# tohinz/multiple-objects-gan

Hardware: AMD Instinct MI355X
Metric: images/sec per G+D train step, 256x256 coco-attngan (higher is better)
Workload: dtype f32

## Files before the change

### include/mogan_hip.h

```cpp
#ifndef MOGAN_HIP_H
#define MOGAN_HIP_H

#include <stddef.h>
#include <stdint.h>

#ifdef __cplusplus
extern "C" {
#endif

typedef struct ihipStream_t* hipStream_t;

#define MOGAN_ERR_SHAPE (-1)
#define MOGAN_ERR_LAUNCH (-2)
#define MOGAN_ERR_WS (-3)

#define MOGAN_ACT_NONE 0
#define MOGAN_ACT_RELU 1
#define MOGAN_ACT_LRELU 2
#define MOGAN_ACT_GLU 3
#define MOGAN_ACT_TANH 4
#define MOGAN_ACT_SIGMOID 5

int mogan_abi_version(void);
int mogan_gemm_set_split_target(int blocks);
// ... 1 lines not shown

int mogan_gemm_tune_set(int mode, int M, int N, int K, int nz, int cfg, int split);
int mogan_gemm_tune_clear(void);

int mogan_reserve_streams(int n);

int mogan_gemm_debug_force(int cfg, int split);
int mogan_gemm_group_min_tiles(int tiles);
int mogan_mfma_form(void);

int mogan_prof_enable(int on);
int mogan_prof_collect(double* out, int max_rows);
int mogan_prof_dump(const char* path);

int mogan_conv2d_out_dims(int Hs, int Ws, int KH, int KW, int stride, int ph, int pw, int up, int* OH, int* OW);
int mogan_conv2d_fwd(const float* x, const float* w, float* y, int B, int Cin, int Hs, int Ws, int Cout, int KH,
                     int KW, int stride, int ph, int pw, int up, void* ws, size_t ws_bytes, hipStream_t stream);
int mogan_logits_head_fwd(const float* x, const float* w, const float* bias, float* p, int B, int K, int Cout,
                          hipStream_t stream);
int mogan_logits_head_bwd(const float* dp, const float* p, const float* x, const float* w, float* dx, float* dw, float* db,
                          int B, int K, int Cout, int accumulate, hipStream_t stream);
int mogan_conv2d_lrelu_fwd(const float* x, const float* w, float* z, int B, int Cin, int Hs, int Ws, int Cout, int KH, int KW,
                           int stride, int ph, int pw, float slope, void* ws, size_t ws_bytes, hipStream_t stream);
int mogan_conv2d_affine_fwd(const float* x, const float* w, const float* scale, const float* shift, float* y, int B,
                            int Cin, int Hs, int Ws, int Cout, int KH, int KW, int stride, int ph, int pw, int relu,
                            void* ws, size_t ws_bytes, hipStream_t stream);
int mogan_affine_relu_bwd_out(const float* y, const float* dy, const float* scale, float* dx, int B, int C, int HW,
                              hipStream_t stream);
typedef struct MoganConvFwdArgs {
    const float* x; long long x_bstride; const float* w; const float* scale; const float* shift;
    float* y; long long y_bstride; float* y2; long long y2_bstride; int msplit;
    int B, Cin, Hs, Ws, Cout, KH, KW, stride, ph, pw, relu;
} MoganConvFwdArgs;
typedef struct MoganConvDgradArgs {
    const float* dy; long long dy_bstride; const float* w; float* dx; long long dx_bstride;
    const float* relu_of; long long relu_bstride; int accumulate;
    int B, Cin, Hs, Ws, Cout, KH, KW, stride, ph, pw;
} MoganConvDgradArgs;
int mogan_conv2d_affine_fwd_group(int n, const MoganConvFwdArgs* args, void* ws, size_t ws_bytes, hipStream_t stream);
int mogan_conv2d_dgrad_group(int n, const MoganConvDgradArgs* args, void* ws, size_t ws_bytes, hipStream_t stream);
int mogan_conv2d_affine_fwd_ex(const float* x, long long x_bstride, const float* w, const float* scale, const float* shift,
                               float* y, long long y_bstride, float* y2, long long y2_bstride, int msplit, int B, int Cin,
                               int Hs, int Ws, int Cout, int KH, int KW, int stride, int ph, int pw, int relu, void* ws,
                               size_t ws_bytes, hipStream_t stream);
int mogan_conv2d_fwd_ex(const float* x, long long x_bstride, const float* w, float* y, long long y_bstride,
                        const float* relu_of, long long relu_bstride, int accumulate, int B, int Cin, int Hs, int Ws,
// ... 295 lines not shown
```

### multiple-objects-gan_amd/csrc/mogan_smallc.hip

```cpp
#include <hip/hip_runtime.h>
#include <stdint.h>
#include <stdlib.h>
#include "../../include/mogan_hip.h"
#include "mogan_internal.h"

namespace {

constexpr int TR = 8, TC = 32;

template <int NC, int NT, int HH, int WW>
__device__ __forceinline__ void halo_load(float (&v)[(NC * HH * WW + NT - 1) / NT], const float* __restrict__ base, size_t plane,
                                          int nvalid, int y0, int x0, int H, int W, int tid) {
    constexpr int TOT = NC * HH * WW, NE = (TOT + NT - 1) / NT;
#pragma unroll
    for (int j = 0; j < NE; ++j) {
        const int e = tid + NT * j;
        const int c = e / (HH * WW), r = e - c * (HH * WW);
        const int hy = r / WW, hx = r - hy * WW;
        const int iy = y0 + hy, ix = x0 + hx;
        const bool ok = e < TOT && c < nvalid && (unsigned)iy < (unsigned)H && (unsigned)ix < (unsigned)W;
        const float t = base[ok ? (size_t)c * plane + (size_t)iy * W + ix : 0];
        v[j] = ok ? t : 0.f;
    }
}
template <int NC, int NT, int HH, int WW, int WP>
__device__ __forceinline__ void halo_store(float (*Xs)[HH][WP], const float (&v)[(NC * HH * WW + NT - 1) / NT], int tid) {
    constexpr int TOT = NC * HH * WW, NE = (TOT + NT - 1) / NT;
#pragma unroll
    for (int j = 0; j < NE; ++j) {
        const int e = tid + NT * j;
        const int c = e / (HH * WW), r = e - c * (HH * WW);
        const int hy = r / WW, hx = r - hy * WW;
        if (e < TOT) Xs[c][hy][hx] = v[j];
    }
}
template <int NC, int NT, int HH, int WW, int WP>
__device__ __forceinline__ void stage_halo(float (*Xs)[HH][WP], const float* __restrict__ base, size_t plane, int nvalid, int y0,
                                           int x0, int H, int W, int tid) {
    float v[(NC * HH * WW + NT - 1) / NT];
    halo_load<NC, NT, HH, WW>(v, base, plane, nvalid, y0, x0, H, W, tid);
    halo_store<NC, NT, HH, WW, WP>(Xs, v, tid);
}

template <int COUT>
// ... 135 lines not shown
    stage_halo<COUT, 256, HH, WW, WP>(Ys, dy + (size_t)b * COUT * plane, plane, COUT, ty * TR - 1, tx * TC - 1, H, W, tid);
    __syncthreads();
    float r[COUT][9];
#pragma unroll
    for (int co = 0; co < COUT; ++co)
#pragma unroll
        for (int kh = 0; kh < 3; ++kh)
#pragma unroll
            for (int kw = 0; kw < 3; ++kw) r[co][kh * 3 + kw] = Ys[co][ly + 2 - kh][lx + 2 - kw];
    const bool inside = iy < H && ix < W;
    float* out = dx + (size_t)b * Cin * plane + (size_t)iy * W + ix;
    for (int ci = 0; ci < Cin; ++ci) {
        float s = 0.f;
#pragma unroll
        for (int co = 0; co < COUT; ++co) {
            const float* wc = w + ((size_t)co * Cin + ci) * 9;
#pragma unroll
            for (int k = 0; k < 9; ++k) s = fmaf(r[co][k], wc[k], s);
        }
        if (inside) out[(size_t)ci * plane] = s;
    }
}

template <int CIN>
__global__ __launch_bounds__(256) void sc_dgrad_k4s2(const float* __restrict__ dy, const float* __restrict__ w,
                                                     float* __restrict__ dx, int Cout, int H, int W, int OH, int OW,
                                                     int tiles_x, int tiles_y) {
    constexpr int CK = 8, HH = TR + 2, WW = TC + 2, WP = WW + 1;
    __shared__ float Ys[CK][HH][WP];
    int t = blockIdx.x;
    const int tx = t % tiles_x; t /= tiles_x;
    const int ty = t % tiles_y; const int b = t / tiles_y;
    const int tid = threadIdx.x, ly = tid >> 5, lx = tid & 31;
    const int Y = ty * TR + ly, X = tx * TC + lx;
    const size_t oplane = (size_t)OH * OW;
    float acc[CIN][2][2];
#pragma unroll
    for (int ci = 0; ci < CIN; ++ci) acc[ci][0][0] = acc[ci][0][1] = acc[ci][1][0] = acc[ci][1][1] = 0.f;
    float pre[(CK * HH * WW + 255) / 256];
    halo_load<CK, 256, HH, WW>(pre, dy + (size_t)b * Cout * oplane, oplane, Cout, ty * TR - 1, tx * TC - 1, OH, OW, tid);
    for (int c0 = 0; c0 < Cout; c0 += CK) {
        halo_store<CK, 256, HH, WW, WP>(Ys, pre, tid);
        __syncthreads();
        if (c0 + CK < Cout)
            halo_load<CK, 256, HH, WW>(pre, dy + ((size_t)b * Cout + c0 + CK) * oplane, oplane, Cout - c0 - CK, ty * TR - 1, tx * TC - 1, OH,
                                       OW, tid);
        const int nc = min(CK, Cout - c0);
        for (int c = 0; c < nc; ++c) {
            float d[3][3];
#pragma unroll
            for (int a = 0; a < 3; ++a)
#pragma unroll
                for (int bb = 0; bb < 3; ++bb) d[a][bb] = Ys[c][ly + a][lx + bb];
            const float* wc = w + (size_t)(c0 + c) * CIN * 16;
#pragma unroll
            for (int ci = 0; ci < CIN; ++ci) {
                const float* k = wc + ci * 16;
#pragma unroll
                for (int py = 0; py < 2; ++py)
#pragma unroll
                    for (int px = 0; px < 2; ++px) {
                        const int kh0 = py ? 0 : 1, a0 = py ? 2 : 1, kh1 = py ? 2 : 3, a1 = py ? 1 : 0;
                        const int kw0 = px ? 0 : 1, b0 = px ? 2 : 1, kw1 = px ? 2 : 3, b1 = px ? 1 : 0;
                        float s = acc[ci][py][px];
                        s = fmaf(d[a0][b0], k[kh0 * 4 + kw0], s);
                        s = fmaf(d[a0][b1], k[kh0 * 4 + kw1], s);
                        s = fmaf(d[a1][b0], k[kh1 * 4 + kw0], s);
                        s = fmaf(d[a1][b1], k[kh1 * 4 + kw1], s);
                        acc[ci][py][px] = s;
// ... 312 lines not shown
        return hipGetLastError() == hipSuccess ? 1 : MOGAN_ERR_LAUNCH;
    }
    if (up != 0 || ph != 1 || pw != 1) return 0;
    if (KH == 3 && KW == 3 && stride == 1 && Cout >= 1 && Cout <= 4) {
        const int tiles_x = cdiv(Ws, TC), tiles_y = cdiv(Hs, TR);
        const long long nb = (long long)B * tiles_x * tiles_y;
        if (nb > 0x7fffffffLL) return 0;
        dim3 grid((unsigned)nb);
        switch (Cout) {
            case 1: hipLaunchKernelGGL(sc_dgrad3x3<1>, grid, dim3(256), 0, st, dy, w, dx, Cin, Hs, Ws, tiles_x, tiles_y); break;
            case 2: hipLaunchKernelGGL(sc_dgrad3x3<2>, grid, dim3(256), 0, st, dy, w, dx, Cin, Hs, Ws, tiles_x, tiles_y); break;
            case 3: hipLaunchKernelGGL(sc_dgrad3x3<3>, grid, dim3(256), 0, st, dy, w, dx, Cin, Hs, Ws, tiles_x, tiles_y); break;
            default: hipLaunchKernelGGL(sc_dgrad3x3<4>, grid, dim3(256), 0, st, dy, w, dx, Cin, Hs, Ws, tiles_x, tiles_y); break;
        }
        return hipGetLastError() == hipSuccess ? 1 : MOGAN_ERR_LAUNCH;
    }
    if (KH == 4 && KW == 4 && stride == 2 && Cin >= 1 && Cin <= 4 && (Hs % 2) == 0 && (Ws % 2) == 0 &&
        (((uintptr_t)dx) & 7) == 0) {
        const int tiles_x = cdiv(OW, TC), tiles_y = cdiv(OH, TR);
        const long long nb = (long long)B * tiles_x * tiles_y;
        if (nb > 0x7fffffffLL) return 0;
        dim3 grid((unsigned)nb);
        switch (Cin) {
            case 1: hipLaunchKernelGGL(sc_dgrad_k4s2<1>, grid, dim3(256), 0, st, dy, w, dx, Cout, Hs, Ws, OH, OW, tiles_x, tiles_y); break;
            case 2: hipLaunchKernelGGL(sc_dgrad_k4s2<2>, grid, dim3(256), 0, st, dy, w, dx, Cout, Hs, Ws, OH, OW, tiles_x, tiles_y); break;
            case 3: hipLaunchKernelGGL(sc_dgrad_k4s2<3>, grid, dim3(256), 0, st, dy, w, dx, Cout, Hs, Ws, OH, OW, tiles_x, tiles_y); break;
            default: hipLaunchKernelGGL(sc_dgrad_k4s2<4>, grid, dim3(256), 0, st, dy, w, dx, Cout, Hs, Ws, OH, OW, tiles_x, tiles_y); break;
        }
        return hipGetLastError() == hipSuccess ? 1 : MOGAN_ERR_LAUNCH;
    }
    return 0;
}

int mogan_smallc_wgrad_try(const float* dy, const float* x, float* dw, const MoganConvShape& g, int accumulate, void* ws,
                           size_t ws_bytes, hipStream_t st) {
    const int B = g.B, Cin = g.Cin, Hs = g.Hs, Ws = g.Ws, Cout = g.Cout, KH = g.KH, KW = g.KW;
    if (is_full_map(g) && (long long)Cout * Cin * KH * KW < (1ll << 30)) {
        const int K = Cin * KH * KW;
        hipLaunchKernelGGL(sc_dot_wgrad, dim3((unsigned)cdiv(Cout * K, 256)), dim3(256), 0, st, dy, x, dw, K, Cout, B, accumulate);
        return hipGetLastError() == hipSuccess ? 1 : MOGAN_ERR_LAUNCH;
    }
    if (!(mogan_is_k33(g) && g.up == 0 && Cout >= 1 && Cout <= 4)) return 0;
    const int tiles_x = cdiv(Ws, TC), tiles_y = cdiv(Hs, TR);
    const long long nblk = (long long)B * tiles_y;
    const int n = Cout * Cin * 9;
    if (nblk > 65535 || !ws || ws_bytes < (size_t)nblk * n * sizeof(float)) return 0;
    float* part = (float*)ws;
    dim3 grid((unsigned)nblk, (unsigned)cdiv(Cin, 8));
    switch (Cout) {
        case 1: hipLaunchKernelGGL(sc_wgrad3x3<1>, grid, dim3(192), 0, st, dy, x, part, Cin, Hs, Ws, tiles_x, tiles_y); break;
        case 2: hipLaunchKernelGGL(sc_wgrad3x3<2>, grid, dim3(192), 0, st, dy, x, part, Cin, Hs, Ws, tiles_x, tiles_y); break;
        case 3: hipLaunchKernelGGL(sc_wgrad3x3<3>, grid, dim3(192), 0, st, dy, x, part, Cin, Hs, Ws, tiles_x, tiles_y); break;
        default: hipLaunchKernelGGL(sc_wgrad3x3<4>, grid, dim3(192), 0, st, dy, x, part, Cin, Hs, Ws, tiles_x, tiles_y); break;
    }
    hipLaunchKernelGGL(sc_wgrad_reduce, dim3((unsigned)cdiv(n, 4)), dim3(256), 0, st, (const float*)part, dw, n, (int)nblk,
                       accumulate);
    return hipGetLastError() == hipSuccess ? 1 : MOGAN_ERR_LAUNCH;
}

extern "C" {

int mogan_logits_head_fwd(const float* x, const float* w, const float* bias, float* p, int B, int K, int Cout,
                          hipStream_t stream) {
    if (!x || !w || !p) return MOGAN_ERR_SHAPE;
    if (B <= 0 || K <= 0 || (K & 3) || Cout < 1 || Cout > 4 || ((((uintptr_t)x) | ((uintptr_t)w)) & 15)) return MOGAN_ERR_SHAPE;
    hipLaunchKernelGGL(logits_head_fwd_kernel, dim3((unsigned)(B * Cout)), dim3(256), 0, stream, x, w, bias, p, K, Cout);
    return hipGetLastError() == hipSuccess ? 0 : MOGAN_ERR_LAUNCH;
}

int mogan_logits_head_bwd(const float* dp, const float* p, const float* x, const float* w, float* dx, float* dw, float* db,
                          int B, int K, int Cout, int accumulate, hipStream_t stream) {
    if (!dp || !p || !x || !w) return MOGAN_ERR_SHAPE;
    if (B <= 0 || K <= 0 || Cout < 1 || Cout > 4 || (long long)B * K >= (1ll << 31)) return MOGAN_ERR_SHAPE;
    const unsigned nbx = dx ? (unsigned)(((long long)B * K + 255) / 256) : 0u;
    const unsigned nbw = dw ? (unsigned)((Cout * K + 255) / 256) : 0u;
    const unsigned nbb = db ? 1u : 0u;
    if (nbx + nbw + nbb == 0) return 0;
    hipLaunchKernelGGL(logits_head_bwd_kernel, dim3(nbx + nbw + nbb), dim3(256), 0, stream, dp, p, x, w, dx, dw, db, B, K, Cout,
                       accumulate, nbx, nbw);
    return hipGetLastError() == hipSuccess ? 0 : MOGAN_ERR_LAUNCH;
}

}
```

### multiple-objects-gan_amd/csrc/mogan_stem.hip

```cpp
#include <hip/hip_runtime.h>
#include <stdint.h>
#include <stdlib.h>
#include <algorithm>
#include "../../include/mogan_hip.h"
#include "mogan_internal.h"
#include "mogan_mma.h"

#if MOGAN_X6
namespace {

typedef float f32x16 __attribute__((ext_vector_type(16)));
typedef float f32x2 __attribute__((ext_vector_type(2)));

template <int TM>
__global__ __launch_bounds__(256, 2) void stem_k4s2_lrelu_kernel(const float* __restrict__ X, const float* __restrict__ w,
                                                              float* __restrict__ Y, int H, int W, int Cout, int OH, int OW,
                                                              float slope, int ngroups, unsigned x_bytes, unsigned y_bytes) {
    constexpr int ROWS = TM * 32;
    __shared__ __attribute__((aligned(16))) uint4 As[3 * 3 * 2 * ROWS];
    const int tid = threadIdx.x, lane = tid & 63, wave = tid >> 6, h = lane >> 5, l31 = lane & 31;
    for (int e = tid; e < ROWS * 3 * 2; e += 256) {
        const int hh = e & 1, c = (e >> 1) % 3, row = e / 6;
        float v[8];
#pragma unroll
// ... 57 lines not shown
        for (int t = 0; t < TM; ++t)
#pragma unroll
            for (int r16 = 0; r16 < 16; ++r16) {
                const int m = t * 32 + (r16 & 3) + 8 * (r16 >> 2);
                float s = acc[t][r16];
                s = s > 0.f ? s : s * slope;
                if (m < Cout) __builtin_amdgcn_raw_buffer_store_b32(__builtin_bit_cast(unsigned, s), rY, vo, (unsigned)m * (unsigned)plane * 4u, 0);
            }
    };
    int g = blockIdx.x * 4 + wave;
    if (g < ngroups) load(g, va);
    while (g < ngroups) {
        const int g1 = g + nwaves;
        if (g1 < ngroups) load(g1, vb);
        compute(g, va);
        if (g1 >= ngroups) break;
        const int g2 = g1 + nwaves;
        if (g2 < ngroups) load(g2, va);
        compute(g1, vb);
        g = g2;
    }
}

}
#endif

int mogan_stem_fwd_try(const float* x, const float* w, float* y, const MoganConvShape& g, float slope, hipStream_t st) {
#if MOGAN_X6
    constexpr int on = 1;
    if (!on) return 0;
    const int B = g.B, H = g.H, W = g.W, Cout = g.Cout, OH = g.OH, OW = g.OW;
    if (!(g.Cin == 3 && mogan_is_k44(g)) || (H & 1) || (W & 1) || B <= 0) return 0;
    if ((OW & 31) || Cout < 32 || Cout > 128 || (Cout & 7) || (((uintptr_t)x) & 7) || !(slope > 0.f)) return 0;
    if ((long long)B * 3 * H * W >= (1ll << 29) || (long long)B * Cout * OH * OW >= (1ll << 30)) return 0;
    const long long ngroups = (long long)B * OH * (OW / 32);
    if (ngroups > 0x7fffffffLL) return 0;
    static int ncu = 0;
    if (!ncu) {
        int dev = 0; hipDeviceProp_t pr;
        if (hipGetDevice(&dev) == hipSuccess && hipGetDeviceProperties(&pr, dev) == hipSuccess) ncu = pr.multiProcessorCount;
        if (ncu <= 0) ncu = 256;
    }
    const int tm = (Cout + 31) / 32;
    const unsigned nblk = (unsigned)std::min<long long>((ngroups + 3) / 4, 2ll * ncu);
    const unsigned xb = 4u * (unsigned)B * 3u * (unsigned)H * (unsigned)W, yb = 4u * (unsigned)B * Cout * OH * OW;
#define MOGAN_STEM_CASE(T) case T: hipLaunchKernelGGL((stem_k4s2_lrelu_kernel<T>), dim3(nblk), dim3(256), 0, st, x, w, y, H, W, Cout, OH, \
                                                      OW, slope, (int)ngroups, xb, yb); break;
    switch (tm) {
// ... 13 lines not shown
```

### multiple-objects-gan_amd/hip/lib.py

```python
import contextlib
import ctypes
import os

import torch

_HERE = os.path.dirname(os.path.dirname(os.path.abspath(__file__)))
LIB_PATH = os.environ.get("MOGAN_LIB") or os.path.join(_HERE, "libmogan_hip.so")

P, I, F, L, Z, D = ctypes.c_void_p, ctypes.c_int, ctypes.c_float, ctypes.c_longlong, ctypes.c_size_t, ctypes.c_double

SIGNATURES = {
    "mogan_abi_version": [],
    "mogan_gemm_set_split_target": [I],
    "mogan_stream_set_split_target": [P, I],
    "mogan_gemm_debug_force": [I, I],
    "mogan_gemm_group_min_tiles": [I],
    "mogan_mfma_form": [],
    "mogan_gemm_tune_set": [I, I, I, I, I, I, I],
    "mogan_gemm_tune_clear": [],
    "mogan_reserve_streams": [ctypes.c_int],
    "mogan_prof_enable": [I],
    "mogan_prof_collect": [P, I],
    "mogan_prof_dump": [ctypes.c_char_p],
    "mogan_conv2d_out_dims": [I, I, I, I, I, I, I, I, P, P],
    "mogan_conv2d_fwd": [P, P, P] + [I] * 11 + [P, Z, P],
    "mogan_logits_head_fwd": [P, P, P, P, I, I, I, P],
    "mogan_logits_head_bwd": [P, P, P, P, P, P, P, I, I, I, I, P],
    "mogan_conv2d_lrelu_fwd": [P, P, P] + [I] * 10 + [F, P, Z, P],
    "mogan_conv2d_affine_fwd": [P, P, P, P, P] + [I] * 11 + [P, Z, P],
    "mogan_affine_relu_bwd_out": [P, P, P, P, I, I, I, P],
    "mogan_conv2d_dgrad": [P, P, P] + [I] * 11 + [P, Z, P],
    "mogan_conv2d_wgrad": [P, P, P] + [I] * 12 + [P, Z, P],
    "mogan_wino_prep_bytes": [I] * 12,
    "mogan_wino_prep_group": [I, P, P, P, P, P, P],
    "mogan_conv_prep_bytes": [I] * 12,
    "mogan_conv_prep_group": [I, P, P, P, P, P, P, P],
    "mogan_conv2d_fwd_wp": [P, P, P, P] + [I] * 11 + [P, Z, P],
    "mogan_conv2d_dgrad_wp": [P, P, P, P] + [I] * 11 + [P, Z, P],
    "mogan_pk_conv_eligible": [I] * 11,
    "mogan_pk_weight_bytes": [I] * 6,
    "mogan_pk_weight_pack": [P, P] + [I] * 8 + [P],
    "mogan_pk_weight_pack_both": [P, P, P] + [I] * 7 + [P],
    "mogan_pk_adam_pack_both": [P] * 7 + [I] * 7 + [F, F, F, F, I, P, I, F, F, I, P],
    "mogan_conv2d_fwd_pk": [P, P, P] + [I] * 10 + [P, Z, P],
    "mogan_conv2d_dgrad_pk": [P, P, P] + [I] * 10 + [P, Z, P],
    "mogan_pk_debug_force": [I, I, I],
    "mogan_pk_wgrad_eligible": [I] * 10 + [Z],
    "mogan_conv2d_wgrad_pk": [P, P, P] + [I] * 11 + [P, Z, P],
    "mogan_pk_panel_bytes": [I, I, I],
    "mogan_deep_block_eligible": [I] * 12,
    "mogan_deep_conv_bn_act_fwd": [P] * 11 + [I] * 10 + [F, F, I, F, I, P, Z, P],
# ... 114 lines not shown
class ConvFwdArgs(ctypes.Structure):
    _fields_ = [("x", P), ("x_bstride", L), ("w", P), ("scale", P), ("shift", P), ("y", P), ("y_bstride", L), ("y2", P),
                ("y2_bstride", L), ("msplit", I)] + [(k, I) for k in ("B", "Cin", "Hs", "Ws", "Cout", "KH", "KW", "stride",
                                                                      "ph", "pw", "relu")]


class ConvDgradArgs(ctypes.Structure):
    _fields_ = [("dy", P), ("dy_bstride", L), ("w", P), ("dx", P), ("dx_bstride", L), ("relu_of", P), ("relu_bstride", L),
                ("accumulate", I)] + [(k, I) for k in ("B", "Cin", "Hs", "Ws", "Cout", "KH", "KW", "stride", "ph", "pw")]


class PkArgs(ctypes.Structure):
    _fields_ = [("wpk", P), ("panel", P), ("raw", P)] + [(k, I) for k in ("B", "M", "Cp", "CGp", "cg0", "PH", "PW", "outH", "outW",
                                                                       "KH", "KW", "stride", "ph", "pw", "dgrad", "nsplit")]


class TailArgs(ctypes.Structure):
    _fields_ = [("src", P * 3), ("src_bs", L * 3), ("src_slab", L * 3), ("src_nsplit", I * 3), ("nsrc", I), ("add", P), ("add_bs", L),
                ("mask", P), ("mask_bs", L), ("scale", P), ("shift", P), ("relu", I), ("box", I), ("dst", P), ("dst_bs", L),
                ("panel", P), ("CGp", I), ("cg0", I), ("B", I), ("n", I), ("H", I), ("W", I)]


_RESTYPE = {"mogan_bn_ws_bytes": Z, "mogan_upconv3x3_ws_bytes": Z, "mogan_pk_weight_bytes": Z, "mogan_pk_panel_bytes": Z,
            "mogan_wino_prep_bytes": Z, "mogan_conv_prep_bytes": Z, "mogan_poly3_mmd_ws_bytes": Z,
            "mogan_knn_sqdist_ws_bytes": Z, "mogan_ball_count_ws_bytes": Z, "mogan_swd_moments_ws_bytes": Z,
            "mogan_ssim_level_ws_bytes": Z, "mogan_knn_cross_ws_bytes": Z, "mogan_radial_power_ws_bytes": Z}
_ERRORS = {-1: "MOGAN_ERR_SHAPE", -2: "MOGAN_ERR_LAUNCH", -3: "MOGAN_ERR_WS"}

_lib = None
_ws = {}
WORKSPACE_BYTES = int(os.environ.get("MOGAN_WS_MB", "256")) << 20


class MoganHipError(RuntimeError):
    pass


def load():
    global _lib
    if _lib is None:
        if not os.path.isfile(LIB_PATH):
            raise MoganHipError(
                "libmogan_hip.so is not built (%s). Run `python __graft_entry__.py` / "
                "`python multiple-objects-gan_amd/build.py`; there is no CPU fallback." % LIB_PATH)
        lib = ctypes.CDLL(LIB_PATH)
        for name, args in SIGNATURES.items():
# ... 112 lines not shown
```

### multiple-objects-gan_amd/hip/ops.py

```python
import contextlib
import ctypes
import os

import torch

from . import lib
from .lib import call, ptr, stream_ptr, workspace

ACT_NONE, ACT_RELU, ACT_LRELU, ACT_GLU, ACT_TANH, ACT_SIGMOID = 0, 1, 2, 3, 4, 5

ACT_TRACE = None


BN_DEFER = None


def bn_apply_deferred(pending):
    for mean, invstd, n, rm, rv, eps, momentum in pending:
        if rm is not None or rv is not None:
            call("mogan_bn_running_update", ptr(mean), ptr(invstd), ptr(rm), ptr(rv), mean.numel(), int(n), float(eps),
                 float(momentum), stream_ptr())
    del pending[:]


# ... 69 lines not shown
    return True


def overwrite_drop(ptrs):
    for p in ptrs:
        _OVERWRITE.pop(p, None)
    del ptrs[:]


def overwrite_stale(g):
    rec = _OVERWRITE.get(g.data_ptr())
    return rec is not None and rec[1] != rec[0][0]


def _first_of_round(g):
    rec = _OVERWRITE.get(g.data_ptr()) if _OVERWRITE else None
    if rec is None:
        return False
    first = rec[1] != rec[0][0]
    rec[1] = rec[0][0]
    return first


def _wgrad_launch(dy, x, w_shape, geom, g):
    stride, ph, pw, up = geom
    acc = not _first_of_round(g)
    if WGRAD_SIDE_STREAM:
        cur, side = _wgrad_stream()
        side.wait_stream(cur)
        with torch.cuda.stream(side):
            conv2d_wgrad(dy, x, w_shape, stride, ph, pw, up, out=g, accumulate=acc)
        fr = _wgrad_frames[-1]
        if side not in fr.used:
            fr.used.append(side)
        fr.keep.append((dy, x))
        _grad_hit(g, side)
    else:
        conv2d_wgrad(dy, x, w_shape, stride, ph, pw, up, out=g, accumulate=acc)
        _grad_hit(g)


def _wgrad_accumulate(dy, x, w, geom, g):
    K = dy.shape[0] * dy.shape[2] * dy.shape[3]
    if not (MERGE_WGRAD and _wgrad_ctx_depth > 0 and K <= _MERGE_K and w.numel() >= _MERGE_W) \
            or (torch.cuda.is_current_stream_capturing() and not MERGE_WGRAD_CAPTURED):
        _wgrad_launch(dy, x, w.shape, geom, g)
        return
    cur = torch.cuda.current_stream()
    key = (g.data_ptr(), cur.cuda_stream)
    prev = _wgrad_pending.pop(key, None)
    if prev is None:
        _wgrad_pending[key] = (dy, x, tuple(w.shape), geom, g, cur)
        _wgrad_frames[-1].parked.append(key)
        return
    pdy, px, _, pgeom = prev[:4]
    if pgeom == geom and pdy.shape[1:] == dy.shape[1:] and px.shape[1:] == x.shape[1:]:
        _wgrad_launch(_cat_batch(pdy, dy), _cat_batch(px, x), w.shape, geom, g)
    else:
        _wgrad_launch(pdy, px, w.shape, pgeom, g)
        _wgrad_launch(dy, x, w.shape, geom, g)


def _cat_batch(a, b):
    a, b = _c(a), _c(b)
    if a.shape[1:] != b.shape[1:]:
# ... 384 lines not shown
        dx = torch.empty((B, Cin, Hs, Ws), dtype=torch.float32, device=dy.device)
        pk = getattr(w, "_mogan_pk", None)
        if pk is not None and WINO_PREP and UPCONV_OWNED:
            k4, img = pk.upconv_pointers(1, B, Hs, Ws)
            call("mogan_conv2d_fwd_wp", ptr(dy), k4, img, ptr(dx), B, Cout, 2 * Hs, 2 * Ws, Cin, 4, 4, 2, 1, 1, 0, wsp, wsn, stream_ptr())
            return dx
        call("mogan_upconv3x3_dgrad", ptr(dy), ptr(w), ptr(dx), B, Cin, Hs, Ws, Cout, wsp, wsn, stream_ptr())
        return dx
    du = torch.empty((B, Cin, Hs << up, Ws << up), dtype=torch.float32, device=dy.device)
    wprep = _wino_prep_ptr(w, 1, B, Hs, Ws, stride, ph, pw, up) if _prep_kind(KH, KW, stride, up) else None
    if wprep is not None:
        call("mogan_conv2d_dgrad_wp", ptr(dy), ptr(w), wprep, ptr(du), B, Cin, Hs, Ws, Cout, KH, KW, stride, ph, pw, up,
             wsp, wsn, stream_ptr())
    else:
        call("mogan_conv2d_dgrad", ptr(dy), ptr(w), ptr(du), B, Cin, Hs, Ws, Cout, KH, KW, stride, ph, pw, up,
             wsp, wsn, stream_ptr())
    if not up:
        return du
    dx = torch.empty((B, Cin, Hs, Ws), dtype=torch.float32, device=dy.device)
    call("mogan_down2_sum", ptr(du), ptr(dx), B * Cin, Hs, Ws, stream_ptr())
    return dx


def conv2d_wgrad(dy, x, w_shape, stride, ph, pw, up, out=None, accumulate=False):
    B, Cin, Hs, Ws = x.shape
    Cout, _, KH, KW = w_shape
    wsp, wsn = workspace(dy.device)
    dw = out if out is not None else torch.empty(w_shape, dtype=torch.float32, device=dy.device)
    if PK_ENABLED and PK_WGRAD and not up:
        key = (B, Cin, Hs, Ws, Cout, KH, KW, stride, ph, pw, wsn)
        e = _pk_wgrad_elig.get(key)
        if e is None:
            e = _pk_wgrad_elig[key] = bool(lib.load().mogan_pk_wgrad_eligible(B, Cin, Hs, Ws, Cout, KH, KW, stride, ph, pw, wsn))
        if e:
            call("mogan_conv2d_wgrad_pk", ptr(dy), ptr(x), ptr(dw), B, Cin, Hs, Ws, Cout, KH, KW, stride, ph, pw,
                 1 if accumulate else 0, wsp, wsn, stream_ptr())
            PK_STATS["wgrad"] = PK_STATS.get("wgrad", 0) + 1
            return dw
    if _is_upconv(w_shape, stride, ph, pw, up):
        call("mogan_upconv3x3_wgrad", ptr(dy), ptr(x), ptr(dw), B, Cin, Hs, Ws, Cout, 1 if accumulate else 0, wsp, wsn,
             stream_ptr())
        return dw
    call("mogan_conv2d_wgrad", ptr(dy), ptr(x), ptr(dw), B, Cin, Hs, Ws, Cout, KH, KW, stride, ph, pw, up,
         1 if accumulate else 0, wsp, wsn, stream_ptr())
    return dw


class Conv2dFn(torch.autograd.Function):

    @staticmethod
    def forward(ctx, x, w, bias, stride, ph, pw, up):
# ... 68 lines not shown
        x, w = _c(x), _c(w)
        B, Cin, Hs, Ws = x.shape
        Cout, _, KH, KW = w.shape
        OH, OW = conv_out_hw(Hs, Ws, KH, KW, stride, ph, pw, 0)
        z = torch.empty((B, Cout, OH, OW), dtype=torch.float32, device=x.device)
        wsp, wsn = workspace(x.device)
        rc = lib.load().mogan_conv2d_lrelu_fwd(ptr(x), ptr(w), ptr(z), B, Cin, Hs, Ws, Cout, KH, KW, stride, ph, pw, slope,
                                               wsp, wsn, stream_ptr())
        if rc == 1:
            z = conv2d_forward(x, w, stride, ph, pw, 0)
            call("mogan_act_fwd", ptr(z), ptr(z), B, Cout, OH * OW, ACT_LRELU, slope, stream_ptr())
        elif rc != 0:
            raise lib.MoganHipError("mogan_conv2d_lrelu_fwd failed: %s" % lib._ERRORS.get(rc, rc))
        if ACT_TRACE is not None:
            _trace(ACT_LRELU, z, TRACE_GROUPS)
        ctx.save_for_backward(x, w, z)
        ctx.cfg = (stride, ph, pw, slope)
        return z

    @staticmethod
    def backward(ctx, dz):
        x, w, z = ctx.saved_tensors
        stride, ph, pw, slope = ctx.cfg
        g = torch.empty_like(z)
        call("mogan_act_bwd", ptr(z), ptr(_c(dz)), ptr(g), z.shape[0], z.shape[1], z.shape[2] * z.shape[3], ACT_LRELU, slope,
             stream_ptr())
        dx = conv2d_dgrad(g, w, x.shape, stride, ph, pw, 0) if ctx.needs_input_grad[0] else None
        dw = None
        if ctx.needs_input_grad[1]:
            gb = _grad_buf(w)
            if gb is not None:
                _wgrad_accumulate(g, x, w, (stride, ph, pw, 0), gb)
            else:
                dw = conv2d_wgrad(g, x, w.shape, stride, ph, pw, 0)
        return dx, dw, None, None, None, None


class LogitsHeadFn(torch.autograd.Function):

    @staticmethod
    def forward(ctx, x, w, bias):
        x, w = _c(x), _c(w)
        B, Cout, K = x.shape[0], w.shape[0], w[0].numel()
        p = torch.empty((B, Cout, 1, 1), dtype=torch.float32, device=x.device)
        call("mogan_logits_head_fwd", ptr(x), ptr(w), ptr(_c(bias)) if bias is not None else None, ptr(p), B, K, Cout,
             stream_ptr())
        ctx.save_for_backward(x, w, p)
        ctx.bias_ref = bias
        return p

    @staticmethod
    def backward(ctx, dp):
        x, w, p = ctx.saved_tensors
        bias = ctx.bias_ref
        B, Cout, K = x.shape[0], w.shape[0], w[0].numel()
        dp = _c(dp)
        dx = torch.empty_like(x) if ctx.needs_input_grad[0] else None
# ... 1540 lines not shown
```

Measured before the change: 455.2.

## Fuse LeakyReLU backward into stem k4s2 conv dgrad and wgrad kernels

Adds a dedicated MFMA-based weight-gradient kernel for the 4x4 stride-2 stem convolution that applies the LeakyReLU mask on the fly from the saved output, plus a masked variant of the small-Cin dgrad kernel. Both read dz and z directly, so the separate activation-backward pass and its intermediate gradient tensor are no longer needed. The wgrad writes per-block partial slabs to workspace and reduces them in a second finish kernel. Eligibility checks fall back to the old path, and the fused dgrad is only used above a size threshold.

```diff
diff --git a/include/mogan_hip.h b/include/mogan_hip.h
--- a/include/mogan_hip.h
+++ b/include/mogan_hip.h
@@ -47,6 +47,11 @@
                           int B, int K, int Cout, int accumulate, hipStream_t stream);
 int mogan_conv2d_lrelu_fwd(const float* x, const float* w, float* z, int B, int Cin, int Hs, int Ws, int Cout, int KH, int KW,
                            int stride, int ph, int pw, float slope, void* ws, size_t ws_bytes, hipStream_t stream);
+size_t mogan_conv2d_k4s2_lrelu_wgrad_ws_bytes(int B, int Cin, int Hs, int Ws, int Cout);
+int mogan_conv2d_k4s2_lrelu_wgrad(const float* dz, const float* z, const float* x, float* dw, int B, int Cin, int Hs, int Ws,
+                                  int Cout, float slope, int accumulate, void* ws, size_t ws_bytes, hipStream_t stream);
+int mogan_conv2d_k4s2_lrelu_dgrad(const float* dz, const float* z, const float* w, float* dx, int B, int Cin, int Hs, int Ws,
+                                  int Cout, float slope, hipStream_t stream);
 int mogan_conv2d_affine_fwd(const float* x, const float* w, const float* scale, const float* shift, float* y, int B,
                             int Cin, int Hs, int Ws, int Cout, int KH, int KW, int stride, int ph, int pw, int relu,
                             void* ws, size_t ws_bytes, hipStream_t stream);
diff --git a/multiple-objects-gan_amd/csrc/mogan_smallc.hip b/multiple-objects-gan_amd/csrc/mogan_smallc.hip
--- a/multiple-objects-gan_amd/csrc/mogan_smallc.hip
+++ b/multiple-objects-gan_amd/csrc/mogan_smallc.hip
@@ -10,7 +10,8 @@
 
 template <int NC, int NT, int HH, int WW>
 __device__ __forceinline__ void halo_load(float (&v)[(NC * HH * WW + NT - 1) / NT], const float* __restrict__ base, size_t plane,
-                                          int nvalid, int y0, int x0, int H, int W, int tid) {
+                                          int nvalid, int y0, int x0, int H, int W, int tid,
+                                          const float* __restrict__ zbase = nullptr, float slope = 1.f) {
     constexpr int TOT = NC * HH * WW, NE = (TOT + NT - 1) / NT;
 #pragma unroll
     for (int j = 0; j < NE; ++j) {
@@ -19,7 +20,9 @@
         const int hy = r / WW, hx = r - hy * WW;
         const int iy = y0 + hy, ix = x0 + hx;
         const bool ok = e < TOT && c < nvalid && (unsigned)iy < (unsigned)H && (unsigned)ix < (unsigned)W;
-        const float t = base[ok ? (size_t)c * plane + (size_t)iy * W + ix : 0];
+        const size_t off = ok ? (size_t)c * plane + (size_t)iy * W + ix : 0;
+        float t = base[off];
+        if (zbase) t = zbase[off] > 0.f ? t : t * slope;
         v[j] = ok ? t : 0.f;
     }
 }
@@ -201,10 +204,11 @@
     }
 }
 
-template <int CIN>
+template <int CIN, bool MASK = false>
 __global__ __launch_bounds__(256) void sc_dgrad_k4s2(const float* __restrict__ dy, const float* __restrict__ w,
                                                      float* __restrict__ dx, int Cout, int H, int W, int OH, int OW,
-                                                     int tiles_x, int tiles_y) {
+                                                     int tiles_x, int tiles_y, const float* __restrict__ z = nullptr,
+                                                     float slope = 1.f) {
     constexpr int CK = 8, HH = TR + 2, WW = TC + 2, WP = WW + 1;
     __shared__ float Ys[CK][HH][WP];
     int t = blockIdx.x;
@@ -217,13 +221,14 @@
 #pragma unroll
     for (int ci = 0; ci < CIN; ++ci) acc[ci][0][0] = acc[ci][0][1] = acc[ci][1][0] = acc[ci][1][1] = 0.f;
     float pre[(CK * HH * WW + 255) / 256];
-    halo_load<CK, 256, HH, WW>(pre, dy + (size_t)b * Cout * oplane, oplane, Cout, ty * TR - 1, tx * TC - 1, OH, OW, tid);
+    halo_load<CK, 256, HH, WW>(pre, dy + (size_t)b * Cout * oplane, oplane, Cout, ty * TR - 1, tx * TC - 1, OH, OW, tid,
+                               MASK ? z + (size_t)b * Cout * oplane : nullptr, slope);
     for (int c0 = 0; c0 < Cout; c0 += CK) {
         halo_store<CK, 256, HH, WW, WP>(Ys, pre, tid);
         __syncthreads();
         if (c0 + CK < Cout)
             halo_load<CK, 256, HH, WW>(pre, dy + ((size_t)b * Cout + c0 + CK) * oplane, oplane, Cout - c0 - CK, ty * TR - 1, tx * TC - 1, OH,
-                                       OW, tid);
+                                       OW, tid, MASK ? z + ((size_t)b * Cout + c0 + CK) * oplane : nullptr, slope);
         const int nc = min(CK, Cout - c0);
         for (int c = 0; c < nc; ++c) {
             float d[3][3];
@@ -582,10 +587,10 @@
         if (nb > 0x7fffffffLL) return 0;
         dim3 grid((unsigned)nb);
         switch (Cin) {
-            case 1: hipLaunchKernelGGL(sc_dgrad_k4s2<1>, grid, dim3(256), 0, st, dy, w, dx, Cout, Hs, Ws, OH, OW, tiles_x, tiles_y); break;
-            case 2: hipLaunchKernelGGL(sc_dgrad_k4s2<2>, grid, dim3(256), 0, st, dy, w, dx, Cout, Hs, Ws, OH, OW, tiles_x, tiles_y); break;
-            case 3: hipLaunchKernelGGL(sc_dgrad_k4s2<3>, grid, dim3(256), 0, st, dy, w, dx, Cout, Hs, Ws, OH, OW, tiles_x, tiles_y); break;
-            default: hipLaunchKernelGGL(sc_dgrad_k4s2<4>, grid, dim3(256), 0, st, dy, w, dx, Cout, Hs, Ws, OH, OW, tiles_x, tiles_y); break;
+            case 1: hipLaunchKernelGGL((sc_dgrad_k4s2<1>), grid, dim3(256), 0, st, dy, w, dx, Cout, Hs, Ws, OH, OW, tiles_x, tiles_y, nullptr, 1.f); break;
+            case 2: hipLaunchKernelGGL((sc_dgrad_k4s2<2>), grid, dim3(256), 0, st, dy, w, dx, Cout, Hs, Ws, OH, OW, tiles_x, tiles_y, nullptr, 1.f); break;
+            case 3: hipLaunchKernelGGL((sc_dgrad_k4s2<3>), grid, dim3(256), 0, st, dy, w, dx, Cout, Hs, Ws, OH, OW, tiles_x, tiles_y, nullptr, 1.f); break;
+            default: hipLaunchKernelGGL((sc_dgrad_k4s2<4>), grid, dim3(256), 0, st, dy, w, dx, Cout, Hs, Ws, OH, OW, tiles_x, tiles_y, nullptr, 1.f); break;
         }
         return hipGetLastError() == hipSuccess ? 1 : MOGAN_ERR_LAUNCH;
     }
@@ -620,6 +625,25 @@
 
 extern "C" {
 
+int mogan_conv2d_k4s2_lrelu_dgrad(const float* dz, const float* z, const float* w, float* dx, int B, int Cin, int Hs, int Ws,
+                                  int Cout, float slope, hipStream_t stream) {
+    if (!dz || !w || !dx) return MOGAN_ERR_SHAPE;
+    if (B <= 0 || Cin <= 0 || Hs <= 0 || Ws <= 0 || Cout <= 0) return MOGAN_ERR_SHAPE;
+    if (Cin > 4 || (Hs & 1) || (Ws & 1) || (((uintptr_t)dx) & 7)) return 1;
+    const int OH = Hs / 2, OW = Ws / 2;
+    const int tiles_x = cdiv(OW, TC), tiles_y = cdiv(OH, TR);
+    const long long nb = (long long)B * tiles_x * tiles_y;
+    if (nb > 0x7fffffffLL) return 1;
+    dim3 grid((unsigned)nb);
+#define MOGAN_SC_DG(C) case C: \
+        if (z) hipLaunchKernelGGL((sc_dgrad_k4s2<C, true>), grid, dim3(256), 0, stream, dz, w, dx, Cout, Hs, Ws, OH, OW, tiles_x, tiles_y, z, slope); \
+        else hipLaunchKernelGGL((sc_dgrad_k4s2<C, false>), grid, dim3(256), 0, stream, dz, w, dx, Cout, Hs, Ws, OH, OW, tiles_x, tiles_y, nullptr, 1.f); \
+        break;
+    switch (Cin) { MOGAN_SC_DG(1) MOGAN_SC_DG(2) MOGAN_SC_DG(3) MOGAN_SC_DG(4) }
+#undef MOGAN_SC_DG
+    return hipGetLastError() == hipSuccess ? 0 : MOGAN_ERR_LAUNCH;
+}
+
 int mogan_logits_head_fwd(const float* x, const float* w, const float* bias, float* p, int B, int K, int Cout,
                           hipStream_t stream) {
     if (!x || !w || !p) return MOGAN_ERR_SHAPE;
diff --git a/multiple-objects-gan_amd/csrc/mogan_stem.hip b/multiple-objects-gan_amd/csrc/mogan_stem.hip
--- a/multiple-objects-gan_amd/csrc/mogan_stem.hip
+++ b/multiple-objects-gan_amd/csrc/mogan_stem.hip
@@ -103,8 +103,223 @@
     }
 }
 
-}
-#endif
+template <int TM, int CIN>
+__global__ __launch_bounds__(256, 1) void stem_k4s2_lrelu_wgrad_kernel(const float* __restrict__ dz, const float* __restrict__ z,
+                                                                    const float* __restrict__ X, float* __restrict__ part, int H, int W,
+                                                                    int OH, int OW, float slope, int nitems, unsigned x_bytes,
+                                                                    unsigned g_bytes) {
+    constexpr int TN = CIN > 2 ? 2 : 1, NV = 16 * CIN, NROW = 4 * CIN, RS = 68, COUT = TM * 32;
+    __shared__ float Ps[4][NROW * RS];
+    __shared__ float Red[COUT * NV];
+    const int tid = threadIdx.x, lane = tid & 63, wave = __builtin_amdgcn_readfirstlane(tid >> 6), h = lane >> 5, l31 = lane & 31;
+    const bool masked = z != nullptr;
+    const __amdgpu_buffer_rsrc_t rX = __builtin_amdgcn_make_buffer_rsrc((void*)X, (short)0, (int)x_bytes, 0x00020000);
+    const __amdgpu_buffer_rsrc_t rD = __builtin_amdgcn_make_buffer_rsrc((void*)dz, (short)0, (int)g_bytes, 0x00020000);
+    const __amdgpu_buffer_rsrc_t rZ = __builtin_amdgcn_make_buffer_rsrc((void*)(masked ? z : dz), (short)0, (int)g_bytes, 0x00020000);
+    const int ipr = OW >> 5, nwaves = gridDim.x * 4;
+    const unsigned plane = (unsigned)OH * (unsigned)OW;
+    float* P = Ps[wave];
+
+    struct Set { uint4 d[TM][2][2], m[TM][2][2]; float xp[NROW + 1]; };
+    Set st[2];
+    const int g0 = blockIdx.x * 4 + wave;
+    const int nmy = g0 < nitems ? (nitems - g0 + nwaves - 1) / nwaves : 0;
+    constexpr unsigned PAST = 0x80000000u;
+    auto load = [&](int j, Set& v) {
+        const bool live = j < nmy;
+        const int g = g0 + j * nwaves;
+        const int oxg = g % ipr; const int r = g / ipr;
+        const int oy = r % OH, b = r / OH;
+        const unsigned va = (((unsigned)(b * COUT + l31)) * plane + (unsigned)oy * OW + (oxg << 5) + 4u * h) * 4u;
+        const unsigned vo = live ? va : PAST, vz = live && masked ? va : PAST;
+#pragma unroll
+        for (int t = 0; t < TM; ++t) {
+            const unsigned so = (unsigned)t * 32u * plane * 4u;
+#pragma unroll
+            for (int s = 0; s < 2; ++s)
+#pragma unroll
+                for (int q = 0; q < 2; ++q) v.d[t][s][q] = __builtin_bit_cast(uint4, __builtin_amdgcn_raw_buffer_load_b128(rD, vo + 32u * (2 * s + q), so, 0));
+#pragma unroll
+            for (int s = 0; s < 2; ++s)
+#pragma unroll
+                for (int q = 0; q < 2; ++q) v.m[t][s][q] = __builtin_bit_cast(uint4, __builtin_amdgcn_raw_buffer_load_b128(rZ, vz + 32u * (2 * s + q), so, 0));
+        }
+#pragma unroll
+        for (int jr = 0; jr <= NROW; ++jr) {
+            const int jj = jr < NROW ? jr : (lane >> 1), c = jr < NROW ? lane : 64 + (lane & 1);
+            const int ci = jj >> 2, iy = 2 * oy - 1 + (jj & 3), ix = (oxg << 6) - 1 + c;
+            const bool ok = live && jj < NROW && (unsigned)iy < (unsigned)H && (unsigned)ix < (unsigned)W;
+            const unsigned idx = ((unsigned)(b * CIN + ci) * H + iy) * W + ix;
+            v.xp[jr] = __builtin_bit_cast(float, __builtin_amdgcn_raw_buffer_load_b32(rX, ok ? idx * 4u : PAST, 0, 0));
+        }
+    };
+    f32x16 acc[TM][TN];
+#pragma unroll
+    for (int t = 0; t < TM; ++t)
+#pragma unroll
+        for (int u = 0; u < TN; ++u)
+#pragma unroll
+            for (int r = 0; r < 16; ++r) acc[t][u][r] = 0.f;
+    auto compute = [&](const Set& v) {
+        __builtin_amdgcn_wave_barrier();
+#pragma unroll
+        for (int j = 0; j < NROW; ++j) P[j * RS + lane] = v.xp[j];
+        if (lane < 2 * NROW) P[(lane >> 1) * RS + 64 + (lane & 1)] = v.xp[NROW];
+        __builtin_amdgcn_s_waitcnt(0xC07F);
+        __builtin_amdgcn_wave_barrier();
+#pragma unroll
+        for (int s = 0; s < 2; ++s) {
+            X6Frag fb[TN];
+#pragma unroll
+            for (int u = 0; u < TN; ++u) {
+                const int n = 32 * u + l31;
+                const bool nv = n < NV;
+                const float* src = P + (nv ? n >> 2 : 0) * RS + (n & 3) + 32 * s + 8 * h;
+                float b8[8];
+#pragma unroll
+                for (int i = 0; i < 8; ++i) { const float t = src[16 * (i >> 2) + 2 * (i & 3)]; b8[i] = nv ? t : 0.f; }
+                fb[u] = x6_split8(b8);
+            }
+#pragma unroll
+            for (int t = 0; t < TM; ++t) {
+                float a8[8];
+#pragma unroll
+                for (int i = 0; i < 8; ++i) {
+                    const uint4 dq = v.d[t][s][i >> 2], mq = v.m[t][s][i >> 2];
+                    const unsigned du = (i & 3) == 0 ? dq.x : (i & 3) == 1 ? dq.y : (i & 3) == 2 ? dq.z : dq.w;
+                    const unsigned mu = (i & 3) == 0 ? mq.x : (i & 3) == 1 ? mq.y : (i & 3) == 2 ? mq.z : mq.w;
+                    const float d = __uint_as_float(du);
+                    a8[i] = masked ? (__uint_as_float(mu) > 0.f ? d : d * slope) : d;
+                }
+                const X6Frag fa = x6_split8(a8);
+#pragma unroll
+                for (int term = 0; term < 6; ++term)
+#pragma unroll
+                    for (int u = 0; u < TN; ++u) acc[t][u] = x6_mfma(fa, fb[u], term, acc[t][u]);
+            }
+        }
+    };
+    load(0, st[0]);
+    for (int j = 0; j < nmy; j += 2) {
+        load(j + 1, st[1]);
+        compute(st[0]);
+        load(j + 2, st[0]);
+        compute(st[1]);
+    }
+#pragma unroll
+    for (int wv = 0; wv < 4; ++wv) {
+        if (wave == wv) {
+#pragma unroll
+            for (int t = 0; t < TM; ++t)
+#pragma unroll
+                for (int u = 0; u < TN; ++u)
+#pragma unroll
+                    for (int r16 = 0; r16 < 16; ++r16) {
+                        const int m = t * 32 + (r16 & 3) + 8 * (r16 >> 2) + 4 * h, n = 32 * u + l31;
+                        if (n < NV) Red[m * NV + n] = wv == 0 ? acc[t][u][r16] : Red[m * NV + n] + acc[t][u][r16];
+                    }
+        }
+        __syncthreads();
+    }
+    float* slab = part + (size_t)blockIdx.x * (COUT * NV);
+    for (int e = tid; e < COUT * NV; e += 256) slab[e] = Red[e];
+}
+
+__global__ __launch_bounds__(256) void stem_wgrad_finish(const float* __restrict__ part, float* __restrict__ dw, int n, int nslab,
+                                                         int accumulate) {
+    __shared__ float S[16][16];
+    const int el = threadIdx.x & 15, p = threadIdx.x >> 4, e = blockIdx.x * 16 + el;
+    const int per = (nslab + 15) >> 4, s0 = p * per, s1 = min(nslab, s0 + per);
+    float s = 0.f;
+    if (e < n)
+        for (int i0 = s0; i0 < s1; i0 += 16) {
+            float v[16];
+#pragma unroll
+            for (int i = 0; i < 16; ++i) v[i] = i0 + i < s1 ? part[(size_t)(i0 + i) * n + e] : 0.f;
+#pragma unroll
+            for (int i = 0; i < 16; ++i) s += v[i];
+        }
+    S[p][el] = s;
+    __syncthreads();
+    if (p == 0 && e < n) {
+        float r = S[0][el];
+#pragma unroll
+        for (int q = 1; q < 16; ++q) r += S[q][el];
+        dw[e] = accumulate ? dw[e] + r : r;
+    }
+}
+
+static int stem_ncu() {
+    static int ncu = 0;
+    if (!ncu) {
+        int dev = 0; hipDeviceProp_t pr;
+        if (hipGetDevice(&dev) == hipSuccess && hipGetDeviceProperties(&pr, dev) == hipSuccess) ncu = pr.multiProcessorCount;
+        if (ncu <= 0) ncu = 256;
+    }
+    return ncu;
+}
+
+}
+#endif
+
+namespace {
+static int stem_wgrad_geom(int B, int Cin, int Hs, int Ws, int Cout) {
+    if (B <= 0 || Cin <= 0 || Hs <= 0 || Ws <= 0 || Cout <= 0) return MOGAN_ERR_SHAPE;
+#if MOGAN_X6
+    if (Cin > 4 || (Cout & 31) || Cout > 128 || (Hs & 1) || (Ws & 1) || ((Ws / 2) & 31)) return 1;
+    if ((long long)B * Cin * Hs * Ws >= (1ll << 29) || (long long)B * Cout * (Hs / 2) * (Ws / 2) >= (1ll << 29)) return 1;
+    return 0;
+#else
+    return 1;
+#endif
+}
+static long long stem_wgrad_items(int B, int Hs, int Ws) { return (long long)B * (Hs / 2) * (Ws / 2 / 32); }
+}
+
+extern "C" {
+
+size_t mogan_conv2d_k4s2_lrelu_wgrad_ws_bytes(int B, int Cin, int Hs, int Ws, int Cout) {
+    if (stem_wgrad_geom(B, Cin, Hs, Ws, Cout) != 0) return 0;
+#if MOGAN_X6
+    const long long nblk = std::min<long long>((stem_wgrad_items(B, Hs, Ws) + 3) / 4, stem_ncu());
+    return (size_t)nblk * Cout * 16 * Cin * sizeof(float);
+#else
+    return 0;
+#endif
+}
+
+int mogan_conv2d_k4s2_lrelu_wgrad(const float* dz, const float* z, const float* x, float* dw, int B, int Cin, int Hs, int Ws,
+                                  int Cout, float slope, int accumulate, void* ws, size_t ws_bytes, hipStream_t stream) {
+    if (!dz || !x || !dw || !ws) return MOGAN_ERR_SHAPE;
+    const int rc = stem_wgrad_geom(B, Cin, Hs, Ws, Cout); if (rc) return rc;
+#if MOGAN_X6
+    if ((((uintptr_t)dz) | ((uintptr_t)z)) & 15) return 1;
+    const int OH = Hs / 2, OW = Ws / 2, n = Cout * 16 * Cin;
+    const long long nitems = stem_wgrad_items(B, Hs, Ws);
+    const int nblk = (int)std::min<long long>((nitems + 3) / 4, stem_ncu());
+    if (ws_bytes < (size_t)nblk * n * sizeof(float)) return MOGAN_ERR_SHAPE;
+    float* part = (float*)ws;
+    const unsigned xb = 4u * (unsigned)B * Cin * Hs * Ws, gb = 4u * (unsigned)B * Cout * OH * OW;
+    mogan_prof_begin(6, 0, 2.0 * n * (double)B * OH * OW, Cout, 16 * Cin, B * OH * OW, stream);
+#define MOGAN_STEM_WG(T, C) case (T) * 8 + (C): hipLaunchKernelGGL((stem_k4s2_lrelu_wgrad_kernel<T, C>), dim3(nblk), dim3(256), 0, stream, \
+                                dz, z, x, part, Hs, Ws, OH, OW, slope, (int)nitems, xb, gb); break;
+    switch ((Cout / 32) * 8 + Cin) {
+        MOGAN_STEM_WG(1, 1) MOGAN_STEM_WG(1, 2) MOGAN_STEM_WG(1, 3) MOGAN_STEM_WG(1, 4)
+        MOGAN_STEM_WG(2, 1) MOGAN_STEM_WG(2, 2) MOGAN_STEM_WG(2, 3) MOGAN_STEM_WG(2, 4)
+        MOGAN_STEM_WG(3, 1) MOGAN_STEM_WG(3, 2) MOGAN_STEM_WG(3, 3) MOGAN_STEM_WG(3, 4)
+        MOGAN_STEM_WG(4, 1) MOGAN_STEM_WG(4, 2) MOGAN_STEM_WG(4, 3) MOGAN_STEM_WG(4, 4)
+    }
+#undef MOGAN_STEM_WG
+    hipLaunchKernelGGL(stem_wgrad_finish, dim3((unsigned)((n + 15) / 16)), dim3(256), 0, stream, (const float*)part, dw, n, nblk,
+                       accumulate);
+    mogan_prof_end(1, stream);
+    return hipGetLastError() == hipSuccess ? 0 : MOGAN_ERR_LAUNCH;
+#else
+    return 1;
+#endif
+}
+
+}
 
 int mogan_stem_fwd_try(const float* x, const float* w, float* y, const MoganConvShape& g, float slope, hipStream_t st) {
 #if MOGAN_X6
diff --git a/multiple-objects-gan_amd/hip/lib.py b/multiple-objects-gan_amd/hip/lib.py
--- a/multiple-objects-gan_amd/hip/lib.py
+++ b/multiple-objects-gan_amd/hip/lib.py
@@ -27,6 +27,9 @@
     "mogan_logits_head_fwd": [P, P, P, P, I, I, I, P],
     "mogan_logits_head_bwd": [P, P, P, P, P, P, P, I, I, I, I, P],
     "mogan_conv2d_lrelu_fwd": [P, P, P] + [I] * 10 + [F, P, Z, P],
+    "mogan_conv2d_k4s2_lrelu_wgrad_ws_bytes": [I] * 5,
+    "mogan_conv2d_k4s2_lrelu_wgrad": [P, P, P, P] + [I] * 5 + [F, I, P, Z, P],
+    "mogan_conv2d_k4s2_lrelu_dgrad": [P, P, P, P] + [I] * 5 + [F, P],
     "mogan_conv2d_affine_fwd": [P, P, P, P, P] + [I] * 11 + [P, Z, P],
     "mogan_affine_relu_bwd_out": [P, P, P, P, I, I, I, P],
     "mogan_conv2d_dgrad": [P, P, P] + [I] * 11 + [P, Z, P],
@@ -187,6 +190,7 @@
 
 
 _RESTYPE = {"mogan_bn_ws_bytes": Z, "mogan_upconv3x3_ws_bytes": Z, "mogan_pk_weight_bytes": Z, "mogan_pk_panel_bytes": Z,
+            "mogan_conv2d_k4s2_lrelu_wgrad_ws_bytes": Z,
             "mogan_wino_prep_bytes": Z, "mogan_conv_prep_bytes": Z, "mogan_poly3_mmd_ws_bytes": Z,
             "mogan_knn_sqdist_ws_bytes": Z, "mogan_ball_count_ws_bytes": Z, "mogan_swd_moments_ws_bytes": Z,
             "mogan_ssim_level_ws_bytes": Z, "mogan_knn_cross_ws_bytes": Z, "mogan_radial_power_ws_bytes": Z}
diff --git a/multiple-objects-gan_amd/hip/ops.py b/multiple-objects-gan_amd/hip/ops.py
--- a/multiple-objects-gan_amd/hip/ops.py
+++ b/multiple-objects-gan_amd/hip/ops.py
@@ -115,25 +115,28 @@
     return first
 
 
-def _wgrad_launch(dy, x, w_shape, geom, g):
+def _wgrad_launch(dy, x, w_shape, geom, g, mask=None):
     stride, ph, pw, up = geom
     acc = not _first_of_round(g)
     if WGRAD_SIDE_STREAM:
         cur, side = _wgrad_stream()
         side.wait_stream(cur)
         with torch.cuda.stream(side):
-            conv2d_wgrad(dy, x, w_shape, stride, ph, pw, up, out=g, accumulate=acc)
+            conv2d_wgrad(dy, x, w_shape, stride, ph, pw, up, out=g, accumulate=acc, mask=mask)
         fr = _wgrad_frames[-1]
         if side not in fr.used:
             fr.used.append(side)
-        fr.keep.append((dy, x))
+        fr.keep.append((dy, x) if mask is None else (dy, x, mask[0]))
         _grad_hit(g, side)
     else:
-        conv2d_wgrad(dy, x, w_shape, stride, ph, pw, up, out=g, accumulate=acc)
+        conv2d_wgrad(dy, x, w_shape, stride, ph, pw, up, out=g, accumulate=acc, mask=mask)
         _grad_hit(g)
 
 
-def _wgrad_accumulate(dy, x, w, geom, g):
+def _wgrad_accumulate(dy, x, w, geom, g, mask=None):
+    if mask is not None:
+        _wgrad_launch(dy, x, w.shape, geom, g, mask)
+        return
     K = dy.shape[0] * dy.shape[2] * dy.shape[3]
     if not (MERGE_WGRAD and _wgrad_ctx_depth > 0 and K <= _MERGE_K and w.numel() >= _MERGE_W) \
             or (torch.cuda.is_current_stream_capturing() and not MERGE_WGRAD_CAPTURED):
@@ -564,11 +567,46 @@
     return dx
 
 
-def conv2d_wgrad(dy, x, w_shape, stride, ph, pw, up, out=None, accumulate=False):
+STEM_BWD = os.environ.get("MOGAN_STEM_BWD", "1") != "0"
+STEM_BWD_STATS = {"wgrad": 0, "dgrad": 0, "act_bwd": 0}
+STEM_BWD_DGRAD_MIN = int(os.environ.get("MOGAN_STEM_BWD_DGRAD_MIN", str(1 << 24)))
+_stem_wgrad_elig = {}
+
+
+def _lrelu_grad(z, dz, slope):
+    g = torch.empty_like(z)
+    call("mogan_act_bwd", ptr(z), ptr(dz), ptr(g), z.shape[0], z.shape[1], z.shape[2] * z.shape[3], ACT_LRELU, slope, stream_ptr())
+    STEM_BWD_STATS["act_bwd"] += 1
+    return g
+
+
+def _stem_wgrad_ok(x, w_shape, geom, dz, z):
+    if not STEM_BWD or tuple(w_shape[2:]) != (4, 4) or tuple(geom) != (2, 1, 1, 0):
+        return False
+    key = tuple(x.shape) + (w_shape[0],)
+    e = _stem_wgrad_elig.get(key)
+    if e is None:
+        e = _stem_wgrad_elig[key] = lib.load().mogan_conv2d_k4s2_lrelu_wgrad_ws_bytes(*key) > 0
+    return e and dz.data_ptr() % 16 == 0 and z.data_ptr() % 16 == 0
+
+
+def conv2d_wgrad(dy, x, w_shape, stride, ph, pw, up, out=None, accumulate=False, mask=None):
     B, Cin, Hs, Ws = x.shape
     Cout, _, KH, KW = w_shape
     wsp, wsn = workspace(dy.device)
     dw = out if out is not None else torch.empty(w_shape, dtype=torch.float32, device=dy.device)
+    if mask is not None:
+        z, slope = mask
+        rc = 1
+        if _stem_wgrad_ok(x, w_shape, (stride, ph, pw, up), dy, z):
+            rc = lib.load().mogan_conv2d_k4s2_lrelu_wgrad(ptr(dy), ptr(z), ptr(x), ptr(dw), B, Cin, Hs, Ws, Cout, slope,
+                                                          1 if accumulate else 0, wsp, wsn, stream_ptr())
+        if rc == 0:
+            STEM_BWD_STATS["wgrad"] += 1
+            return dw
+        if rc != 1:
+            raise lib.MoganHipError("mogan_conv2d_k4s2_lrelu_wgrad failed: %s" % lib._ERRORS.get(rc, rc))
+        dy = _lrelu_grad(z, dy, slope)
     if PK_ENABLED and PK_WGRAD and not up:
         key = (B, Cin, Hs, Ws, Cout, KH, KW, stride, ph, pw, wsn)
         e = _pk_wgrad_elig.get(key)
@@ -683,17 +721,37 @@
     def backward(ctx, dz):
         x, w, z = ctx.saved_tensors
         stride, ph, pw, slope = ctx.cfg
-        g = torch.empty_like(z)
-        call("mogan_act_bwd", ptr(z), ptr(_c(dz)), ptr(g), z.shape[0], z.shape[1], z.shape[2] * z.shape[3], ACT_LRELU, slope,
-             stream_ptr())
-        dx = conv2d_dgrad(g, w, x.shape, stride, ph, pw, 0) if ctx.needs_input_grad[0] else None
+        dz = _c(dz)
+        geom = (stride, ph, pw, 0)
+        g = []
+
+        def masked_dz():
+            if not g:
+                g.append(_lrelu_grad(z, dz, slope))
+            return g[0]
+
+        dx = None
+        if ctx.needs_input_grad[0]:
+            rc = 1
+            if STEM_BWD and tuple(w.shape[2:]) == (4, 4) and geom == (2, 1, 1, 0) and z.numel() >= STEM_BWD_DGRAD_MIN:
+                dx = torch.empty_like(x)
+                rc = lib.load().mogan_conv2d_k4s2_lrelu_dgrad(ptr(dz), ptr(z), ptr(w), ptr(dx), x.shape[0], x.shape[1], x.shape[2],
+                                                              x.shape[3], w.shape[0], slope, stream_ptr())
+            if rc == 0:
+                STEM_BWD_STATS["dgrad"] += 1
+            elif rc == 1:
+                dx = conv2d_dgrad(masked_dz(), w, x.shape, stride, ph, pw, 0)
+            else:
+                raise lib.MoganHipError("mogan_conv2d_k4s2_lrelu_dgrad failed: %s" % lib._ERRORS.get(rc, rc))
         dw = None
         if ctx.needs_input_grad[1]:
+            fused = _stem_wgrad_ok(x, w.shape, geom, dz, z)
+            dy, mask = (dz, (z, slope)) if fused else (masked_dz(), None)
             gb = _grad_buf(w)
             if gb is not None:
-                _wgrad_accumulate(g, x, w, (stride, ph, pw, 0), gb)
+                _wgrad_accumulate(dy, x, w, geom, gb, mask)
             else:
-                dw = conv2d_wgrad(g, x, w.shape, stride, ph, pw, 0)
+                dw = conv2d_wgrad(dy, x, w.shape, stride, ph, pw, 0, mask=mask)
         return dx, dw, None, None, None, None
 
 
```

New measurement: 457.8, median of 6. About the same (+0.6%).
